# OneWalkman/EDGE-YOLO

Hardware: AMD Instinct MI355X
Metric: images/sec @ 640x640 fp16 (EdgeLine-YOLO detection forward path: backbone + DWT neck + GFLv2 head decode + batched NMS) (higher is better)
Workload: dtype f16; 1 GPU; yolo11n-test.yaml (scale n, nc=80) predict path, 640x640, batch 32/GPU, conf 0.25 iou 0.7 max_det 300, random-init weights, default head biases (DENSE NMS regime: mean detections/img 300); regime=dense, global_batch=32, imgsz=640, nc=80

## Files before the change

edge-yolo_amd/_lib.py:

```python
import ctypes as C
import os

import torch

_HERE = os.path.dirname(os.path.abspath(__file__))
LIB_PATH = os.path.join(_HERE, "csrc", "libedgeyolo_hip.so")

F16, F32 = 0, 1
ACT_NONE, ACT_SILU, ACT_RELU, ACT_SIGMOID = 0, 1, 2, 3
ATTN_AREA_F32, ATTN_AREA_F16, ATTN_AREA_MFMA = 401, 402, 403


class HipLibraryError(RuntimeError):
    pass


class ConvDesc(C.Structure):
    _fields_ = [
        ("dtype", C.c_int32), ("B", C.c_int32), ("H", C.c_int32), ("W", C.c_int32), ("Ho", C.c_int32), ("Wo", C.c_int32),
        ("Cout", C.c_int32), ("k", C.c_int32), ("stride", C.c_int32), ("pad", C.c_int32), ("act", C.c_int32), ("nsrc", C.c_int32),
        ("src", C.c_void_p * 2), ("src_C", C.c_int32 * 2), ("src_cstride", C.c_int32 * 2), ("src_up", C.c_int32 * 2),
        ("w", C.c_void_p), ("bias", C.c_void_p), ("y", C.c_void_p), ("y_cstride", C.c_int32),
        ("res", C.c_void_p), ("res_cstride", C.c_int32), ("out_scale", C.c_float),
        ("addz", C.c_void_p), ("addz_cstride", C.c_int32), ("addz_H", C.c_int32), ("addz_W", C.c_int32), ("ngroup", C.c_int32),
# ... 23 lines not shown
        ("ngroup", C.c_int32), ("src_g", C.c_int64), ("y_g", C.c_int64), ("heads", C.c_int32),
        ("kpad", C.c_int32), ("nt_pack", C.c_int32), ("mt", C.c_int32), ("nti", C.c_int32), ("lds", C.c_int32), ("tile_nti", C.c_int32), ("tile_src_lds", C.c_int32 * 2), ("tile_src_lcs", C.c_int32 * 2), ("tile_y_lds", C.c_int32), ("tile_y_lcs", C.c_int32), ("tile_res_lds", C.c_int32), ("tile_res_lcs", C.c_int32), ("tile_lds_bytes", C.c_int32), ("zsy", C.c_float), ("zsx", C.c_float),
    ]


BLK_CONV, BLK_DW, BLK_DWT, BLK_POOL, BLK_LINATTN = range(5)
_vp, _i, _f, _sz = C.c_void_p, C.c_int, C.c_float, C.c_size_t
SIGNATURES = {
    "ey_last_error": (C.c_char_p, []),
    "ey_version": (_i, []),
    "ey_abi_sizeof": (_sz, [_i]),
    "ey_tune_set": (_i, [C.c_char_p, C.c_long]),
    "ey_tune_get": (C.c_long, [C.c_char_p]),
    "ey_conv_packed_bytes": (_sz, [_i, _i, _i, _i]),
    "ey_conv_pack_weight": (_i, [_i, _i, _i, _i, _vp, _vp, _sz]),
    "ey_conv2d": (_i, [C.POINTER(ConvDesc), _vp]),
    "ey_conv_pw_pair": (_i, [C.POINTER(ConvDesc), C.POINTER(ConvDesc), _vp]),
    "ey_conv_variant": (_i, [_i, _i, _i, _i, _i, _i, C.c_long, _i]),
    "ey_conv_last_variant": (_i, []),
    "ey_conv_pack_nt": (_i, [_i]),
    "ey_conv_chain_klen": (_i, [_i]),
    "ey_conv_chain_kperm": (_i, [_i, _vp, _i]),
    "ey_conv_pw_chain": (_i, [_i, _i, _i, _i, _i, _i, _i, _vp, _i, _vp, _vp, _i, _vp, _vp, _i, _vp, _i, _vp]),
    "ey_conv2d_direct": (_i, [C.POINTER(ConvDirectDesc), _vp]),
    "ey_stem_conv": (_i, [_i, _i, _i, _i, _i, _i, _i, _i, _vp, _vp, _vp, _vp, _i, _vp]),
    "ey_dwconv": (_i, [_i, _i, _i, _i, _i, _i, _i, _vp, _i, _vp, _vp, _vp, _i, _vp]),
    "ey_dsconv": (_i, [_i, _i, _i, _i, _i, _i, _i, _i, _vp, _i, _vp, _vp, _i, _vp, _vp, _vp, _i, _vp, _i, _vp]),
    "ey_dsconv_toeplitz_bytes": (_sz, [_i, _i]),
    "ey_dsconv_pack_toeplitz": (_i, [_i, _i, _vp, _vp, _sz]),
    "ey_dsconv_tz": (_i, [_i, _i, _i, _i, _i, _i, _i, _i, _vp, _i, _vp, _vp, _vp, _i, _vp, _vp, _vp, _i, _vp, _i, _vp]),
    "ey_dsconv_last_variant": (_i, []),
    "ey_conv_pw_conv3s2": (_i, [_i, _i, _i, _i, _vp, _i, _i, _vp, _i, _i, _i, _vp, _vp, _i, _i, _vp, _vp, _i, _vp, _i, _vp]),
    "ey_stem_pair": (_i, [_i, _i, _i, _vp, _vp, _vp, _i, _i, _vp, _vp, _i, _vp, _i, _vp]),
    "ey_dsb_pair": (_i, [_i, _i, _i, _i, _i, _i, _i, _i, _vp, _i, _vp, _vp, _vp, _vp, _vp, _vp, _i, _vp, _i, _vp]),
    "ey_dwt_haar": (_i, [_i, _i, _i, _i, _i, _vp, _i, _vp, _i, _vp]),
    "ey_dwt": (_i, [_i, _i, _i, _i, _i, _i, _vp, _vp, _i, _vp, _i, _vp]),
    "ey_wavelet_z": (_i, [_i, _i, _i, _i, _i, _vp, _i, _vp, C.c_long, _vp, _vp, _vp, _i, _vp]),
    "ey_wavelet_z2": (_i, [_i, _i, _i, _i, _i, _i, _vp, _i, _vp, _vp, _i, _vp, C.c_long, _vp, _vp, _vp, _i, _vp]),
    "ey_sppf_pool": (_i, [_i, _i, _i, _i, _i, _vp, _i, _vp, _vp, _vp, _i, _vp]),
    "ey_copy_nhwc": (_i, [_i, _i, _i, _i, _i, _i, _vp, _i, _vp, _i, _vp]),
    "ey_scale_add_channels": (_i, [_i, _i, _i, _i, _i, _vp, _i, _vp, _vp, _i, _vp, _i, _vp]),
    "ey_avgpool2": (_i, [_i, _i, _i, _i, _i, _vp, _i, _vp, _i, _vp]),
    "ey_dwconv_s2": (_i, [_i, _i, _i, _i, _i, _i, _i, _vp, _i, _vp, _vp, _vp, _i, _vp]),
    "ey_hypergraph_workspace_bytes": (_sz, [_i, _i, _i, _i]),
    "ey_hypergraph_conv": (_i, [_i, _i, _i, _i, _i, _i, _i, _vp, _i, _vp, _i, _vp, _vp, _vp, _vp, _vp, _vp, _vp, _vp, _vp, _vp, _sz, _vp]),
    "ey_nchw_to_nhwc": (_i, [_i, _i, _i, _i, _i, _vp, _vp, _i, _vp]),
    "ey_nhwc_to_nchw": (_i, [_i, _i, _i, _i, _i, _vp, _i, _vp, _vp]),
    "ey_letterbox": (_i, [_i, _vp, _i, _i, _i, _vp, _i, _i, _i, _i, _i, _i, _i, _i, _vp]),
    "ey_copy_linear": (_i, [_vp, _vp, _sz, _vp]),
    "ey_letterbox_batch": (_i, [_i, _vp, _i, _i, _i, _i, C.c_long, _vp, _i, _i, _i, _i, _i, _i, _i, _i, _vp]),
    "ey_linear_attention": (_i, [_i, _i, _i, _i, _i, _vp, _i, _vp, _i, _vp]),
    "ey_softmax_attention": (_i, [_i, _i, _i, _i, _i, _i, _f, _vp, _i, _vp, _i, _vp]),
    "ey_attention_last_variant": (_i, []),
    "ey_area_attention": (_i, [_i, _i, _i, _i, _i, _i, _f, _vp, _i, _vp, _i, _vp, _i, _vp, _i, _vp]),
    "ey_head_decode_last_variant": (_i, []),
    "ey_head_decode": (_i, [_i, _i, _i, _i, _i, _f, _vp, _i, _vp, _i, _vp, _vp, _vp, _vp, _i, _vp, _i, _i, _vp]),
    "ey_head_decode_levels": (_i, [_i, _i, _i, _vp, _vp, _vp, _vp, _vp, _vp, _vp, _i, _vp, _vp, _vp, _vp, _i, _vp, _i, _vp, _vp]),
    "ey_head_decode_levels_xyxy": (_i, [_i, _i, _i, _vp, _vp, _vp, _vp, _vp, _vp, _vp, _i, _vp, _vp, _vp, _vp, _i, _vp, _i, _vp, _vp]),
    "ey_e2e_topk_workspace_bytes": (_sz, [_i, _i, _i]),
    "ey_e2e_topk": (_i, [_i, _i, _i, _vp, _i, _vp, _vp, _vp, _sz, _vp]),
    "ey_block_stage_sizeof": (_sz, []),
    "ey_block_program_bytes": (_sz, [_i]),
    "ey_block_compile": (_i, [C.POINTER(BlockStage), _i, _vp, _sz]),
    "ey_block_run": (_i, [_vp, _i, _i, C.POINTER(C.c_void_p), _i, _vp]),
    "ey_block_tileable": (_i, [C.POINTER(BlockStage), _i]),
    "ey_block_run_tiles": (_i, [_vp, _i, _i, _i, _i, _i, C.POINTER(C.c_void_p), _i, _vp]),
# ... 108 lines not shown
```

edge-yolo_amd/csrc/api.cpp:

```cpp
#include <stdarg.h>
#include <stdio.h>
#include <stddef.h>
#include <string.h>
#include "../../include/edgeyolo_hip.h"
#include "tune.h"

static thread_local char g_err[512] = "";

int ey_set_error(int code, const char* fmt, ...) {
  va_list ap;
  va_start(ap, fmt);
  vsnprintf(g_err, sizeof(g_err), fmt, ap);
  va_end(ap);
  return code;
}

extern "C" const char* ey_last_error(void) { return g_err; }
extern "C" int ey_version(void) { return 1; }
extern "C" size_t ey_abi_sizeof(int which) { return which == 0 ? sizeof(ey_conv_desc) : which == 1 ? sizeof(ey_conv_direct_desc) : 0; }

EyTune g_ey_tune;
#define EY_T(f) {#f, offsetof(EyTune, f)}
static const struct { const char* name; size_t off; } k_tunables[] = {
    EY_T(tiles_per_wave), EY_T(mt2_min_m), EY_T(small_m), EY_T(small_wmb), EY_T(halo_min_c), EY_T(ws_lds_kb), EY_T(ws_wg_cu), EY_T(ws_k3_minnt), EY_T(tile_wlds),
    EY_T(tile_s2_minc), EY_T(tile_s2_minm), EY_T(grid_div), EY_T(c3r), EY_T(tile_minwg), EY_T(tile_flat), EY_T(tile_mink), EY_T(pwr_m), EY_T(pwr_frags), EY_T(pw_m),
    EY_T(pw_waves), EY_T(pw_wmb), EY_T(ds_p), EY_T(tz_kmask), EY_T(tz_minpx), EY_T(ds_strip), EY_T(stem_mfma), EY_T(linattn_mfma), EY_T(softattn_mfma), EY_T(areaattn_mfma), EY_T(c3p), EY_T(c3p_min_m), EY_T(c3p_fast), EY_T(c3s), EY_T(c3s_mt4_m), EY_T(c3s_min_work), EY_T(c3s_cfg), EY_T(nms_fast_k), EY_T(nms_mask_wg), EY_T(sppf_min_wg), EY_T(sppf_cv), EY_T(dsb_pair), EY_T(dsb_max_px), EY_T(dsb_rb), EY_T(dsb_fixed), EY_T(dsb_p2), EY_T(stem_pair), EY_T(pw3), EY_T(pw3_min_px), EY_T(pw3_skew), EY_T(pwn), EY_T(pwn_max_m), EY_T(pwn_ntw), EY_T(pwc), EY_T(xcd_map), EY_T(nms_mask_k)};
static long* tunable(const char* name) {
  if (!name) return nullptr;
  for (const auto& t : k_tunables)
    if (!strcmp(t.name, name)) return (long*)((char*)&g_ey_tune + t.off);
  return nullptr;
}
extern "C" int ey_tune_set(const char* name, long value) {
  long* p = tunable(name);
  if (!p) return ey_set_error(EY_EINVAL, "ey_tune_set: unknown tunable '%s'", name ? name : "(null)");
  *p = value;
  return EY_OK;
}
extern "C" long ey_tune_get(const char* name) {
  const long* p = tunable(name);
  return p ? *p : -1;
}
```

edge-yolo_amd/csrc/dsb.hip:

```cpp
#include "common.h"
#include "tune.h"

struct DsbP {
  int B, H, W, act, add;
  const void* x; int xCs; unsigned xBytes;
  const void* wdw1; const void* wpw1; const float* b1;
  const void* wdw2; const void* wpw2; const float* b2;
  void* y; int yCs;
  int RB, Kpad;
};

#define DSB_SLACK 8

template <int K, int KS, int P, bool LAST>
__device__ __forceinline__ void dsb_stage(const DsbP& p, int b, const f16* s_src, int srcW, int src_row0, const f16* s_w, const void* wpw, const float* bias_g,
                                          int row_lo, int row_hi, f16* s_dst, int dstW, int dst_row0, int dst_pad, const f16* s_res, int resW, int res_row0,
                                          int res_pad) {
  constexpr int C = 32 * KS, NT = 2 * KS, CP = C + 8, NX = P + K - 1;
  const int lane = threadIdx.x & 63, r = lane & 15, g = lane >> 4, wave = threadIdx.x >> 6, nwave = blockDim.x >> 6;
  const int ch0 = g * 4 * NT;
  Vec8<f16> af[KS][NT];
  {
    const __amdgpu_buffer_rsrc_t rw = ey_rsrc(wpw, (unsigned)(16 * NT * p.Kpad * (int)sizeof(f16)));
    const unsigned wvoff = (unsigned)((r * p.Kpad + 8 * g) * (int)sizeof(f16));
#pragma unroll
    for (int ks = 0; ks < KS; ++ks)
#pragma unroll
      for (int nt = 0; nt < NT; ++nt) BufLoad8<f16>::load(af[ks][nt], rw, wvoff, (nt * 16 * p.Kpad + ks * 32) * (int)sizeof(f16));
  }
  float bias[4 * NT];
#pragma unroll
  for (int i = 0; i < 4 * NT; ++i) bias[i] = bias_g ? bias_g[ch0 + i] : 0.f;
  const int WS = (p.W + P - 1) / P;
  const int nstrip = (row_hi - row_lo) * WS;
  for (int unit = wave; unit * 16 < nstrip; unit += nwave) {
    const int si = unit * 16 + r;
    const bool sv = si < nstrip;
    const int sic = sv ? si : nstrip - 1;
    const int ry = sic / WS, x0 = (sic - ry * WS) * P, oy = row_lo + ry;
    Vec8<f16> bf[KS][P];
#pragma unroll
    for (int ks = 0; ks < KS; ++ks) {
      const int cb = ks * 32 + 8 * g;
      float acc[P][8];
#pragma unroll
      for (int q = 0; q < P; ++q)
#pragma unroll
        for (int i = 0; i < 8; ++i) acc[q][i] = 0.f;
      const f16* base = s_src + ((oy - K / 2 - src_row0) * srcW + x0) * CP + cb;
#pragma unroll
      for (int ky = 0; ky < K; ++ky) {
        Vec8<f16> xr[NX];
#pragma unroll
        for (int j = 0; j < NX; ++j) xr[j].load(base + (ky * srcW + j) * CP);
#pragma unroll
        for (int kx = 0; kx < K; ++kx) {
          Vec8<f16> w;
          w.load(s_w + (ky * K + kx) * C + cb);
#pragma unroll
          for (int q = 0; q < P; ++q) ey_fma8_mix(xr[q + kx], w, acc[q]);
        }
      }
#pragma unroll
      for (int q = 0; q < P; ++q)
#pragma unroll
        for (int i = 0; i < 8; ++i) bf[ks][q].set(i, acc[q][i]);
    }
#pragma unroll
    for (int q = 0; q < P; ++q) {
      f32x4 pacc[NT];
#pragma unroll
      for (int nt = 0; nt < NT; ++nt) pacc[nt] = (f32x4)0.f;
#pragma unroll
      for (int ks = 0; ks < KS; ++ks)
#pragma unroll
        for (int nt = 0; nt < NT; ++nt) pacc[nt] = __builtin_amdgcn_mfma_f32_16x16x32_f16(af[ks][nt].v, bf[ks][q].v, pacc[nt], 0, 0, 0);
      const int ox = x0 + q;
      if (!sv || ox >= p.W) continue;
      float v[4 * NT];
#pragma unroll
      for (int nt = 0; nt < NT; ++nt)
#pragma unroll
        for (int j = 0; j < 4; ++j) v[4 * nt + j] = pacc[nt][j] + bias[4 * nt + j];
      ey_act_n(v, p.act);
      if constexpr (!LAST) {
        f16* d = s_dst + ((oy - dst_row0) * dstW + ox + dst_pad) * CP + ch0;
#pragma unroll
        for (int h = 0; h < NT / 2; ++h) {
          Vec8<f16> o;
#pragma unroll
          for (int j = 0; j < 8; ++j) o.set(j, v[8 * h + j]);
          o.store(d + 8 * h);
        }
      } else {
        const long m = ((long)b * p.H + oy) * p.W + ox;
        f16* yp = (f16*)p.y + m * p.yCs + ch0;
        const f16* rp = s_res + ((oy - res_row0) * resW + ox + res_pad) * CP + ch0;
#pragma unroll
        for (int h = 0; h < NT / 2; ++h) {
          if (p.add) {
            Vec8<f16> rr;
            rr.load(rp + 8 * h);
#pragma unroll
            for (int j = 0; j < 8; ++j) v[8 * h + j] += rr.get(j);
          }
          Vec8<f16> o;
#pragma unroll
          for (int j = 0; j < 8; ++j) o.set(j, v[8 * h + j]);
          o.store(yp + 8 * h);
        }
      }
    }
  }
}

template <int K1, int K2, int KS, int P1, int P2>
__global__ __launch_bounds__(512) void dsb_pair_kernel(DsbP p) {
  extern __shared__ __attribute__((aligned(16))) char smem[];
  constexpr int C = 32 * KS, CP = C + 8, CV = C / 8, R1 = K1 / 2, R2 = K2 / 2, PPI = 512 / CV;
  const int RI = p.RB + 2 * (R1 + R2), WI = p.W + 2 * R1, RM = p.RB + 2 * R2, WM = p.W + 2 * R2;
  f16* s_in = reinterpret_cast<f16*>(smem);
  f16* s_mid = s_in + (RI * WI + DSB_SLACK) * CP;
  f16* s_w1 = s_mid + (RM * WM + DSB_SLACK) * CP;
  f16* s_w2 = s_w1 + K1 * K1 * C;
  const int tid = threadIdx.x, b = blockIdx.y, y0 = blockIdx.x * p.RB;
  {
    const __amdgpu_buffer_rsrc_t rx = ey_rsrc(p.x, p.xBytes);
    const int cv = tid % CV, NP = RI * WI, iy0 = y0 - R1 - R2;
    constexpr int U = 4;
    int base = tid / CV;
    bool first = true;
    do {
      Vec8<f16> t[U];
#pragma unroll
      for (int j = 0; j < U; ++j) {
        const int px = base + j * PPI, trow = px / WI, u = px - trow * WI, iy = iy0 + trow, ix = u - R1;
        const bool ok = px < NP && iy >= 0 && iy < p.H && ix >= 0 && ix < p.W;
        BufLoad8<f16>::load(t[j], rx, ok ? (unsigned)((((b * p.H + iy) * p.W + ix) * p.xCs + cv * 8) * (int)sizeof(f16)) : EY_OOB);
      }
      if (first) {
        first = false;
        Vec8<f16> z;
        z.zero();
        for (int v = tid; v < (RM * WM + DSB_SLACK) * CP / 8; v += 512) z.store(s_mid + v * 8);
        for (int v = tid; v < K1 * K1 * CV; v += 512) {
          Vec8<f16> w;
          w.load((const f16*)p.wdw1 + v * 8);
          w.store(s_w1 + v * 8);
        }
        for (int v = tid; v < K2 * K2 * CV; v += 512) {
          Vec8<f16> w;
          w.load((const f16*)p.wdw2 + v * 8);
          w.store(s_w2 + v * 8);
        }
      }
#pragma unroll
      for (int j = 0; j < U; ++j) {
        const int px = base + j * PPI;
        if (px < NP) t[j].store(s_in + px * CP + cv * 8);
      }
      base += U * PPI;
    } while (base < NP);
  }
  __syncthreads();
  {
    const int lo = y0 - R2 < 0 ? 0 : y0 - R2, hi = y0 + p.RB + R2 > p.H ? p.H : y0 + p.RB + R2;
    dsb_stage<K1, KS, P1, false>(p, b, s_in, WI, y0 - R1 - R2, s_w1, p.wpw1, p.b1, lo, hi, s_mid, WM, y0 - R2, R2, nullptr, 0, 0, 0);
  }
  __syncthreads();
  {
    const int hi = y0 + p.RB > p.H ? p.H : y0 + p.RB;
    dsb_stage<K2, KS, P2, true>(p, b, s_mid, WM, y0 - R2, s_w2, p.wpw2, p.b2, y0, hi, nullptr, 0, 0, 0, s_in, WI, y0 - R1 - R2, R1);
  }
}

static size_t dsb_lds_bytes(int W, int C, int k1, int k2, int RB) {
  const int CP = C + 8, r1 = k1 / 2, r2 = k2 / 2;
  return ((size_t)((RB + 2 * (r1 + r2)) * (W + 2 * r1) + DSB_SLACK) + (size_t)((RB + 2 * r2) * (W + 2 * r2) + DSB_SLACK)) * CP * 2 + (size_t)(k1 * k1 + k2 * k2) * C * 2;
}

static int dsb_band_rows(int B, int H, int W, int C, int k1, int k2) {
  static int ncu = 0;
  if (!ncu) {
    int dev = 0;
    hipDeviceProp_t prop;
    if (hipGetDevice(&dev) == hipSuccess && hipGetDeviceProperties(&prop, dev) == hipSuccess) ncu = prop.multiProcessorCount;
    if (ncu < 1) ncu = 256;
  }
  long force = tune().dsb_rb;
  if (force > H) force = H;
  if (force > 0) return dsb_lds_bytes(W, C, k1, k2, (int)force) <= 160 * 1024 ? (int)force : 0;
  int best = 0;
  double best_cost = 0;
  for (int rb = 1; rb <= H; ++rb) {
    if (dsb_lds_bytes(W, C, k1, k2, rb) > 160 * 1024) break;
    const long wgs = (long)B * ((H + rb - 1) / rb);
    const double rounds = (double)((wgs + ncu - 1) / ncu);
    const double cost = rounds * ((rb + 2 * (k2 / 2)) * k1 * k1 + rb * k2 * k2 + (double)tune().dsb_fixed);
    if (!best || cost < best_cost) best = rb, best_cost = cost;
  }
  return best;
}

template <int K1, int K2, int KS, int P1, int P2>
static int dsb_launch(DsbP p, int bands, size_t lds, hipStream_t st) {
  static size_t reserved = 0;
  if (lds > 64 * 1024 && lds > reserved) {
    if (hipFuncSetAttribute((const void*)dsb_pair_kernel<K1, K2, KS, P1, P2>, hipFuncAttributeMaxDynamicSharedMemorySize, (int)lds) != hipSuccess)
      return ey_set_error(EY_ELAUNCH, "dsb_pair: cannot reserve %zu B of LDS", lds);
    reserved = lds;
  }
  hipLaunchKernelGGL((dsb_pair_kernel<K1, K2, KS, P1, P2>), dim3((unsigned)bands, (unsigned)p.B), dim3(512), lds, st, p);
  EY_LAUNCH_CHECK("ey_dsb_pair");
  return EY_OK;
}

extern "C" int ey_dsb_pair(int dtype, int B, int H, int W, int C, int k1, int k2, int act, const void* x, int x_cstride, const void* w_dw1_kkc,
                           const void* w_pw1_packed, const float* bias1, const void* w_dw2_kkc, const void* w_pw2_packed, const float* bias2, int add_residual,
                           void* y, int y_cstride, ey_stream_t stream) {
  EY_CHECK(x && y && w_dw1_kkc && w_pw1_packed && w_dw2_kkc && w_pw2_packed, "dsb_pair: null pointer");
  EY_CHECK(B > 0 && H > 0 && W > 0, "dsb_pair: bad extent");
  EY_CHECK(x_cstride >= C && y_cstride >= C, "dsb_pair: cstride");
  const int es = 2;
  const long xbytes = (((long)B * H * W - 1) * x_cstride + C) * es, ybytes = (((long)B * H * W - 1) * y_cstride + C) * es;
  const bool fits = tune().dsb_pair && dtype == EY_F16 && (C == 32 || C == 64) && k1 == 3 && (k2 == 5 || k2 == 7) && B <= 65535 && xbytes < (1L << 31) &&
                    ybytes < (1L << 31) && (x_cstride * es) % 16 == 0 && ey_aligned(x, 16) && (y_cstride * es) % 16 == 0 && ey_aligned(y, 16) &&
                    ey_aligned(w_dw1_kkc, 16) && ey_aligned(w_dw2_kkc, 16) && ey_aligned(w_pw1_packed, 16) && ey_aligned(w_pw2_packed, 16) &&
                    (long)B * H * W <= tune().dsb_max_px;
  if (!fits) return ey_set_error(EY_EUNSUPPORTED, "dsb_pair: shape outside the fused kernel (f16, C 32/64, k 3 -> 5/7, small maps)");
  const int RB = dsb_band_rows(B, H, W, C, k1, k2);
  if (RB < 1) return ey_set_error(EY_EUNSUPPORTED, "dsb_pair: a one-row band of a %d-wide map does not fit LDS", W);
  DsbP p;
  p.B = B; p.H = H; p.W = W; p.act = act; p.add = add_residual;
  p.x = x; p.xCs = x_cstride; p.xBytes = (unsigned)xbytes;
  p.wdw1 = w_dw1_kkc; p.wpw1 = w_pw1_packed; p.b1 = bias1; p.wdw2 = w_dw2_kkc; p.wpw2 = w_pw2_packed; p.b2 = bias2;
  p.y = y; p.yCs = y_cstride;
  p.RB = RB; p.Kpad = ey_conv_kpad(C, es);
  const int bands = (H + RB - 1) / RB;
  const size_t lds = dsb_lds_bytes(W, C, k1, k2, RB);
  hipStream_t st = (hipStream_t)stream;
  int P2 = (int)tune().dsb_p2;
  if (P2 != 1 && P2 != 2 && P2 != 4) P2 = RB * ((W + 1) / 2) < 64 ? 1 : 2;
#define DSB(KV, KSV)                                                          \
  if (k2 == KV && C == 32 * KSV) {                                            \
    if (P2 == 1) return dsb_launch<3, KV, KSV, 2, 1>(p, bands, lds, st);      \
    if (P2 == 4) return dsb_launch<3, KV, KSV, 2, 4>(p, bands, lds, st);      \
    return dsb_launch<3, KV, KSV, 2, 2>(p, bands, lds, st);                   \
  }
  DSB(5, 1) DSB(7, 1) DSB(5, 2) DSB(7, 2)
#undef DSB
  return ey_set_error(EY_EINVAL, "dsb_pair: k2=%d C=%d", k2, C);
}
```

edge-yolo_amd/csrc/tune.h:

```cpp
#pragma once
struct EyTune {
  long tiles_per_wave = 0;
  long mt2_min_m = 300000;
  long small_m = 100000;
  long small_wmb = 48;
  long halo_min_c = 48;
  long ws_lds_kb = 76;
  long ws_wg_cu = 2;
  long ws_k3_minnt = 0;
  long tile_wlds = 1;
  long tile_s2_minc = 64;
  long tile_s2_minm = 40000;
  long grid_div = 1;
  long c3p = 1;
  long c3p_min_m = 40000;
  long c3p_fast = 1;
  long c3s = 1;
  long c3s_mt4_m = 100000;
  long c3s_min_work = 20000;
  long c3s_cfg = 0;
  long c3r = 1;
  long tile_minwg = 400;
  long tile_flat = 1;
  long tile_mink = 0;
  long pwr_m = 110000;
  long pwr_frags = 24;
  long pw_m = 110000;
  long pw_waves = 3072;
  long pw_wmb = 64;
  long xcd_map = 31;
  long pwc = 1;
  long pwn = 1;
  long pwn_max_m = 110000;
  long pwn_ntw = 0;
  long ds_p = 0;
  long tz_kmask = 168;
  long tz_minpx = 100000;
  long ds_strip = 1;
  long dsb_pair = 1;
  long dsb_max_px = 300000;
  long dsb_rb = 0;
  long dsb_p2 = 0;
  long dsb_fixed = 100;
  long stem_pair = 1;
  long pw3 = 1;
  long pw3_skew = 8;
  long pw3_min_px = 100000;
  long stem_mfma = 1;
  long linattn_mfma = 1;
  long softattn_mfma = 1;
  long areaattn_mfma = 1;
  long sppf_min_wg = 128;
  long sppf_cv = 0;
  long nms_mask_wg = 0;
  long nms_mask_k = 1536;
  long nms_fast_k = 2048;
};
extern EyTune g_ey_tune;
static inline const EyTune& tune() { return g_ey_tune; }
```

include/edgeyolo_hip.h:

```cpp
#ifndef EDGEYOLO_HIP_H
#define EDGEYOLO_HIP_H
#include <stddef.h>
#include <stdint.h>

#ifdef __cplusplus
extern "C" {
#endif

typedef void* ey_stream_t;

enum { EY_F16 = 0, EY_F32 = 1 };
enum { EY_ACT_NONE = 0, EY_ACT_SILU = 1, EY_ACT_RELU = 2, EY_ACT_SIGMOID = 3 };
enum { EY_OK = 0, EY_EINVAL = -1, EY_EUNSUPPORTED = -2, EY_ELAUNCH = -3 };

const char* ey_last_error(void);
int ey_version(void);
size_t ey_abi_sizeof(int which);
int ey_tune_set(const char* name, long value);
long ey_tune_get(const char* name);

typedef struct {
  int32_t dtype;
  int32_t B, H, W;
  int32_t Ho, Wo;
// ... 40 lines not shown
  const float* w_oihw; const float* bias;
  void* y; int32_t y_cstride;
} ey_conv_direct_desc;
int ey_conv2d_direct(const ey_conv_direct_desc* d, ey_stream_t stream);

int ey_stem_conv(int x_dtype, int y_dtype, int B, int Cin, int H, int W, int Cout, int act, const void* x_nchw,
                 const float* w_oihw, const float* bias, void* y, int y_cstride, ey_stream_t stream);

int ey_conv_pw_pair(const ey_conv_desc* first, const ey_conv_desc* second, ey_stream_t stream);

int ey_conv_pw_conv3s2(int dtype, int B, int H, int W, const void* src0, int C0, int cstride0, const void* src1, int C1, int cstride1, int Cmid,
                       const void* w1_packed, const float* bias1, int act1, int Cout, const void* w2_packed, const float* bias2, int act2, void* y,
                       int y_cstride, ey_stream_t stream);

int ey_stem_pair(int B, int H, int W, const void* x_nchw, const float* w0_oihw, const float* bias0, int act0, int C1, const void* w1_packed,
                 const float* bias1, int act1, void* y, int y_cstride, ey_stream_t stream);

int ey_dwconv(int dtype, int B, int H, int W, int C, int k, int act, const void* x, int x_cstride, const void* w_kkc,
              const float* bias, void* y, int y_cstride, ey_stream_t stream);

int ey_dsconv(int dtype, int B, int H, int W, int Cin, int Cout, int k, int act, const void* x, int x_cstride,
              const void* w_dw_kkc, const float* dw_bias, int dw_act, const void* w_pw_packed, const float* bias, void* y, int y_cstride, const void* res,
              int res_cstride, ey_stream_t stream);

size_t ey_dsconv_toeplitz_bytes(int C, int k);
int ey_dsconv_pack_toeplitz(int C, int k, const float* w_dw_kkc_host, void* out_host, size_t out_bytes);
int ey_dsconv_tz(int dtype, int B, int H, int W, int Cin, int Cout, int k, int act, const void* x, int x_cstride,
                 const void* w_dw_kkc, const void* w_dw_toeplitz, const float* dw_bias, int dw_act, const void* w_pw_packed, const float* bias,
                 void* y, int y_cstride, const void* res, int res_cstride, ey_stream_t stream);

int ey_dsb_pair(int dtype, int B, int H, int W, int C, int k1, int k2, int act, const void* x, int x_cstride, const void* w_dw1_kkc,
                const void* w_pw1_packed, const float* bias1, const void* w_dw2_kkc, const void* w_pw2_packed, const float* bias2, int add_residual,
                void* y, int y_cstride, ey_stream_t stream);

int ey_dsconv_last_variant(void);

int ey_dwt_haar(int dtype, int B, int H, int W, int C, const void* x, int x_cstride, void* y, int y_cstride,
                ey_stream_t stream);

int ey_dwt(int dtype, int B, int H, int W, int C, int k, const float* taps, const void* x, int x_cstride, void* y, int y_cstride,
           ey_stream_t stream);

int ey_wavelet_z(int dtype, int B, int H, int W, int C, const void* x, int x_cstride, const void* w_sub_packed, long w_set_stride, const float* b_sub,
                 const void* w_z_packed, void* z, int z_cstride, ey_stream_t stream);
int ey_wavelet_z2(int dtype, int B, int H, int W, int C, int k, const float* taps, int use_ds, const void* w_dw_kkc, const void* x, int x_cstride,
                  const void* w_sub_packed, long w_set_stride, const float* b_sub, const void* w_z_packed, void* z, int z_cstride, ey_stream_t stream);

int ey_sppf_pool(int dtype, int B, int H, int W, int C, const void* x, int x_cstride, void* y1, void* y2, void* y3,
                 int y_cstride, ey_stream_t stream);

int ey_scale_add_channels(int dtype, int B, int H, int W, int C, const void* x, int x_cstride, const float* gamma, const void* t, int t_cstride,
                          void* y, int y_cstride, ey_stream_t stream);

int ey_avgpool2(int dtype, int B, int H, int W, int C, const void* x, int x_cstride, void* y, int y_cstride, ey_stream_t stream);

int ey_dwconv_s2(int dtype, int B, int H, int W, int C, int k, int act, const void* x, int x_cstride, const void* w_kkc, const float* bias,
                 void* y, int y_cstride, ey_stream_t stream);

size_t ey_hypergraph_workspace_bytes(int B, int N, int D, int E);
int ey_hypergraph_conv(int dtype, int B, int N, int D, int E, int heads, int context, const void* x, int x_cstride, void* y, int y_cstride,
                       const float* proto_base, const float* ctx_wT, const float* ctx_b, const float* pre_w, const float* pre_b,
                       const float* edge_wT, const float* edge_b, const void* node_w, const float* node_b, void* workspace,
                       size_t workspace_bytes, ey_stream_t stream);

int ey_copy_nhwc(int dtype, int B, int H, int W, int C, int up, const void* src, int src_cstride, void* dst,
                 int dst_cstride, ey_stream_t stream);
// ... 97 lines not shown
```

Baseline: 28110 images/s.

## Add column-tiled walking-window DSB kernel with ring-buffered LDS and cost planner

Result: no change. 27990 images/s (-0.4%).

```diff
diff --git a/edge-yolo_amd/_lib.py b/edge-yolo_amd/_lib.py
--- a/edge-yolo_amd/_lib.py
+++ b/edge-yolo_amd/_lib.py
@@ -79,6 +79,7 @@
     "ey_dsconv_last_variant": (_i, []),
     "ey_conv_pw_conv3s2": (_i, [_i, _i, _i, _i, _vp, _i, _i, _vp, _i, _i, _i, _vp, _vp, _i, _i, _vp, _vp, _i, _vp, _i, _vp]),
     "ey_stem_pair": (_i, [_i, _i, _i, _vp, _vp, _vp, _i, _i, _vp, _vp, _i, _vp, _i, _vp]),
+    "ey_dsb_pair_plan": (_i, [_i, _i, _i, _i, _i, _vp]),
     "ey_dsb_pair": (_i, [_i, _i, _i, _i, _i, _i, _i, _i, _vp, _i, _vp, _vp, _vp, _vp, _vp, _vp, _i, _vp, _i, _vp]),
     "ey_dwt_haar": (_i, [_i, _i, _i, _i, _i, _vp, _i, _vp, _i, _vp]),
     "ey_dwt": (_i, [_i, _i, _i, _i, _i, _i, _vp, _vp, _i, _vp, _i, _vp]),
diff --git a/edge-yolo_amd/csrc/api.cpp b/edge-yolo_amd/csrc/api.cpp
--- a/edge-yolo_amd/csrc/api.cpp
+++ b/edge-yolo_amd/csrc/api.cpp
@@ -24,7 +24,7 @@
 static const struct { const char* name; size_t off; } k_tunables[] = {
     EY_T(tiles_per_wave), EY_T(mt2_min_m), EY_T(small_m), EY_T(small_wmb), EY_T(halo_min_c), EY_T(ws_lds_kb), EY_T(ws_wg_cu), EY_T(ws_k3_minnt), EY_T(tile_wlds),
     EY_T(tile_s2_minc), EY_T(tile_s2_minm), EY_T(grid_div), EY_T(c3r), EY_T(tile_minwg), EY_T(tile_flat), EY_T(tile_mink), EY_T(pwr_m), EY_T(pwr_frags), EY_T(pw_m),
-    EY_T(pw_waves), EY_T(pw_wmb), EY_T(ds_p), EY_T(tz_kmask), EY_T(tz_minpx), EY_T(ds_strip), EY_T(stem_mfma), EY_T(linattn_mfma), EY_T(softattn_mfma), EY_T(areaattn_mfma), EY_T(c3p), EY_T(c3p_min_m), EY_T(c3p_fast), EY_T(c3s), EY_T(c3s_mt4_m), EY_T(c3s_min_work), EY_T(c3s_cfg), EY_T(nms_fast_k), EY_T(nms_mask_wg), EY_T(sppf_min_wg), EY_T(sppf_cv), EY_T(dsb_pair), EY_T(dsb_max_px), EY_T(dsb_rb), EY_T(dsb_fixed), EY_T(dsb_p2), EY_T(stem_pair), EY_T(pw3), EY_T(pw3_min_px), EY_T(pw3_skew), EY_T(pwn), EY_T(pwn_max_m), EY_T(pwn_ntw), EY_T(pwc), EY_T(xcd_map), EY_T(nms_mask_k)};
+    EY_T(pw_waves), EY_T(pw_wmb), EY_T(ds_p), EY_T(tz_kmask), EY_T(tz_minpx), EY_T(ds_strip), EY_T(stem_mfma), EY_T(linattn_mfma), EY_T(softattn_mfma), EY_T(areaattn_mfma), EY_T(c3p), EY_T(c3p_min_m), EY_T(c3p_fast), EY_T(c3s), EY_T(c3s_mt4_m), EY_T(c3s_min_work), EY_T(c3s_cfg), EY_T(nms_fast_k), EY_T(nms_mask_wg), EY_T(sppf_min_wg), EY_T(sppf_cv), EY_T(dsb_pair), EY_T(dsb_max_px), EY_T(dsb_rb), EY_T(dsb_fixed), EY_T(dsb_form), EY_T(dsb_tw), EY_T(dsb_sr), EY_T(dsb_thr), EY_T(dsb_p2), EY_T(stem_pair), EY_T(pw3), EY_T(pw3_min_px), EY_T(pw3_skew), EY_T(pwn), EY_T(pwn_max_m), EY_T(pwn_ntw), EY_T(pwc), EY_T(xcd_map), EY_T(nms_mask_k)};
 static long* tunable(const char* name) {
   if (!name) return nullptr;
   for (const auto& t : k_tunables)
diff --git a/edge-yolo_amd/csrc/dsb.hip b/edge-yolo_amd/csrc/dsb.hip
--- a/edge-yolo_amd/csrc/dsb.hip
+++ b/edge-yolo_amd/csrc/dsb.hip
@@ -1,5 +1,6 @@
 #include "common.h"
 #include "tune.h"
+#include <string.h>
 
 struct DsbP {
   int B, H, W, act, add;
@@ -8,36 +9,50 @@
   const void* wdw2; const void* wpw2; const float* b2;
   void* y; int yCs;
   int RB, Kpad;
+  int TW, SR;
 };
 
 #define DSB_SLACK 8
 
-template <int K, int KS, int P, bool LAST>
-__device__ __forceinline__ void dsb_stage(const DsbP& p, int b, const f16* s_src, int srcW, int src_row0, const f16* s_w, const void* wpw, const float* bias_g,
-                                          int row_lo, int row_hi, f16* s_dst, int dstW, int dst_row0, int dst_pad, const f16* s_res, int resW, int res_row0,
-                                          int res_pad) {
+struct DsbTile {
+  f16* s;
+  int W, row0, col0, rows;
+};
+
+template <int KS>
+struct DsbW {
+  Vec8<f16> af[KS][2 * KS];
+  float bias[8 * KS];
+  __device__ __forceinline__ void load(const DsbP& p, const void* wpw, const float* bias_g) {
+    constexpr int NT = 2 * KS;
+    const int lane = threadIdx.x & 63, r = lane & 15, g = lane >> 4;
+    const __amdgpu_buffer_rsrc_t rw = ey_rsrc(wpw, (unsigned)(16 * NT * p.Kpad * (int)sizeof(f16)));
+    const unsigned wvoff = (unsigned)((r * p.Kpad + 8 * g) * (int)sizeof(f16));
+#pragma unroll
+    for (int ks = 0; ks < KS; ++ks)
+#pragma unroll
+      for (int nt = 0; nt < NT; ++nt) BufLoad8<f16>::load(af[ks][nt], rw, wvoff, (nt * 16 * p.Kpad + ks * 32) * (int)sizeof(f16));
+#pragma unroll
+    for (int i = 0; i < 4 * NT; ++i) bias[i] = bias_g ? bias_g[g * 4 * NT + i] : 0.f;
+  }
+};
+
+template <int K, int KS, int P, bool LAST, bool RING>
+__device__ __forceinline__ void dsb_stage(const DsbP& p, int b, const DsbTile src, const f16* s_w, const DsbW<KS>& pw, int row_lo, int row_hi, int col_lo,
+                                          int col_hi, const DsbTile dst, const DsbTile res) {
   constexpr int C = 32 * KS, NT = 2 * KS, CP = C + 8, NX = P + K - 1;
   const int lane = threadIdx.x & 63, r = lane & 15, g = lane >> 4, wave = threadIdx.x >> 6, nwave = blockDim.x >> 6;
   const int ch0 = g * 4 * NT;
-  Vec8<f16> af[KS][NT];
-  {
-    const __amdgpu_buffer_rsrc_t rw = ey_rsrc(wpw, (unsigned)(16 * NT * p.Kpad * (int)sizeof(f16)));
-    const unsigned wvoff = (unsigned)((r * p.Kpad + 8 * g) * (int)sizeof(f16));
-#pragma unroll
-    for (int ks = 0; ks < KS; ++ks)
-#pragma unroll
-      for (int nt = 0; nt < NT; ++nt) BufLoad8<f16>::load(af[ks][nt], rw, wvoff, (nt * 16 * p.Kpad + ks * 32) * (int)sizeof(f16));
-  }
-  float bias[4 * NT];
-#pragma unroll
-  for (int i = 0; i < 4 * NT; ++i) bias[i] = bias_g ? bias_g[ch0 + i] : 0.f;
-  const int WS = (p.W + P - 1) / P;
+  const int srcW = src.W;
+  const int WS = (col_hi - col_lo + P - 1) / P;
   const int nstrip = (row_hi - row_lo) * WS;
   for (int unit = wave; unit * 16 < nstrip; unit += nwave) {
     const int si = unit * 16 + r;
     const bool sv = si < nstrip;
     const int sic = sv ? si : nstrip - 1;
-    const int ry = sic / WS, x0 = (sic - ry * WS) * P, oy = row_lo + ry;
+    const int ry = sic / WS, x0 = col_lo + (sic - ry * WS) * P, oy = row_lo + ry;
+    int srow = oy - K / 2 - src.row0;
+    if constexpr (RING) srow %= src.rows;
     Vec8<f16> bf[KS][P];
 #pragma unroll
     for (int ks = 0; ks < KS; ++ks) {
@@ -47,12 +62,17 @@
       for (int q = 0; q < P; ++q)
 #pragma unroll
         for (int i = 0; i < 8; ++i) acc[q][i] = 0.f;
-      const f16* base = s_src + ((oy - K / 2 - src_row0) * srcW + x0) * CP + cb;
+      const f16* base = src.s + ((RING ? 0 : srow * srcW) + x0 - K / 2 - src.col0) * CP + cb;
 #pragma unroll
       for (int ky = 0; ky < K; ++ky) {
         Vec8<f16> xr[NX];
-#pragma unroll
-        for (int j = 0; j < NX; ++j) xr[j].load(base + (ky * srcW + j) * CP);
+        int trow = ky;
+        if constexpr (RING) {
+          trow = srow + ky;
+          if (trow >= src.rows) trow -= src.rows;
+        }
+#pragma unroll
+        for (int j = 0; j < NX; ++j) xr[j].load(base + (trow * srcW + j) * CP);
 #pragma unroll
         for (int kx = 0; kx < K; ++kx) {
           Vec8<f16> w;
@@ -74,17 +94,19 @@
 #pragma unroll
       for (int ks = 0; ks < KS; ++ks)
 #pragma unroll
-        for (int nt = 0; nt < NT; ++nt) pacc[nt] = __builtin_amdgcn_mfma_f32_16x16x32_f16(af[ks][nt].v, bf[ks][q].v, pacc[nt], 0, 0, 0);
+        for (int nt = 0; nt < NT; ++nt) pacc[nt] = __builtin_amdgcn_mfma_f32_16x16x32_f16(pw.af[ks][nt].v, bf[ks][q].v, pacc[nt], 0, 0, 0);
       const int ox = x0 + q;
-      if (!sv || ox >= p.W) continue;
+      if (!sv || ox >= col_hi) continue;
       float v[4 * NT];
 #pragma unroll
       for (int nt = 0; nt < NT; ++nt)
 #pragma unroll
-        for (int j = 0; j < 4; ++j) v[4 * nt + j] = pacc[nt][j] + bias[4 * nt + j];
+        for (int j = 0; j < 4; ++j) v[4 * nt + j] = pacc[nt][j] + pw.bias[4 * nt + j];
       ey_act_n(v, p.act);
       if constexpr (!LAST) {
-        f16* d = s_dst + ((oy - dst_row0) * dstW + ox + dst_pad) * CP + ch0;
+        int drow = oy - dst.row0;
+        if constexpr (RING) drow %= dst.rows;
+        f16* d = dst.s + (drow * dst.W + ox - dst.col0) * CP + ch0;
 #pragma unroll
         for (int h = 0; h < NT / 2; ++h) {
           Vec8<f16> o;
@@ -95,7 +117,9 @@
       } else {
         const long m = ((long)b * p.H + oy) * p.W + ox;
         f16* yp = (f16*)p.y + m * p.yCs + ch0;
-        const f16* rp = s_res + ((oy - res_row0) * resW + ox + res_pad) * CP + ch0;
+        int rrow = oy - res.row0;
+        if constexpr (RING) rrow %= res.rows;
+        const f16* rp = res.s + (rrow * res.W + ox - res.col0) * CP + ch0;
 #pragma unroll
         for (int h = 0; h < NT / 2; ++h) {
           if (p.add) {
@@ -124,6 +148,7 @@
   f16* s_w1 = s_mid + (RM * WM + DSB_SLACK) * CP;
   f16* s_w2 = s_w1 + K1 * K1 * C;
   const int tid = threadIdx.x, b = blockIdx.y, y0 = blockIdx.x * p.RB;
+  const DsbTile t_in = {s_in, WI, y0 - R1 - R2, -R1, RI}, t_mid = {s_mid, WM, y0 - R2, -R2, RM};
   {
     const __amdgpu_buffer_rsrc_t rx = ey_rsrc(p.x, p.xBytes);
     const int cv = tid % CV, NP = RI * WI, iy0 = y0 - R1 - R2;
@@ -165,12 +190,132 @@
   __syncthreads();
   {
     const int lo = y0 - R2 < 0 ? 0 : y0 - R2, hi = y0 + p.RB + R2 > p.H ? p.H : y0 + p.RB + R2;
-    dsb_stage<K1, KS, P1, false>(p, b, s_in, WI, y0 - R1 - R2, s_w1, p.wpw1, p.b1, lo, hi, s_mid, WM, y0 - R2, R2, nullptr, 0, 0, 0);
+    DsbW<KS> pw;
+    pw.load(p, p.wpw1, p.b1);
+    dsb_stage<K1, KS, P1, false, false>(p, b, t_in, s_w1, pw, lo, hi, 0, p.W, t_mid, t_mid);
   }
   __syncthreads();
   {
     const int hi = y0 + p.RB > p.H ? p.H : y0 + p.RB;
-    dsb_stage<K2, KS, P2, true>(p, b, s_mid, WM, y0 - R2, s_w2, p.wpw2, p.b2, y0, hi, nullptr, 0, 0, 0, s_in, WI, y0 - R1 - R2, R1);
+    DsbW<KS> pw;
+    pw.load(p, p.wpw2, p.b2);
+    dsb_stage<K2, KS, P2, true, false>(p, b, t_mid, s_w2, pw, y0, hi, 0, p.W, t_mid, t_in);
+  }
+}
+
+#define DSB_WALK_PF 4
+template <int K1, int K2, int KS, int P1, int P2>
+__global__ __launch_bounds__(512) void dsb_walk_kernel(DsbP p) {
+  extern __shared__ __attribute__((aligned(16))) char smem[];
+  constexpr int C = 32 * KS, CP = C + 8, CV = C / 8, R1 = K1 / 2, R2 = K2 / 2, RH = R1 + R2;
+  const int RS = p.RB, RI = RS + 2 * RH, WI = p.TW + 2 * RH, RM = RS + 2 * R2, WM = p.TW + 2 * R2;
+  f16* s_in = reinterpret_cast<f16*>(smem);
+  f16* s_mid = s_in + (RI * WI + DSB_SLACK) * CP;
+  f16* s_w1 = s_mid + (RM * WM + DSB_SLACK) * CP;
+  f16* s_w2 = s_w1 + K1 * K1 * C;
+  const int tid = threadIdx.x, nthr = blockDim.x, PPI = nthr / CV, cv = tid % CV;
+  const int nsx = (p.W + p.TW - 1) / p.TW, nsy = (p.H + p.SR - 1) / p.SR;
+  const int wi = (int)ey_xcd_block(blockIdx.x, gridDim.x);
+  const int b = wi / (nsx * nsy), ws = wi - b * (nsx * nsy), sy = ws / nsx;
+  const int x0 = (ws - sy * nsx) * p.TW, y0 = sy * p.SR;
+  const int x1 = x0 + p.TW > p.W ? p.W : x0 + p.TW, y1 = y0 + p.SR > p.H ? p.H : y0 + p.SR;
+  const DsbTile t_in = {s_in, WI, y0 - RH, x0 - RH, RI}, t_mid = {s_mid, WM, y0 - R2, x0 - R2, RM};
+  const __amdgpu_buffer_rsrc_t rx = ey_rsrc(p.x, p.xBytes);
+  auto src_off = [&](int px, int np, int row0, int& lds) -> unsigned {
+    const int trow = px / WI, u = px - trow * WI, iy = row0 + trow, ix = x0 - RH + u;
+    lds = (((iy - t_in.row0) % RI) * WI + u) * CP + cv * 8;
+    const bool ok = px < np && iy >= 0 && iy < p.H && ix >= 0 && ix < p.W;
+    return ok ? (unsigned)((((b * p.H + iy) * p.W + ix) * p.xCs + cv * 8) * (int)sizeof(f16)) : EY_OOB;
+  };
+  {
+    const int NP = RI * WI;
+    constexpr int U = 4;
+    int base = tid / CV;
+    bool first = true;
+    do {
+      Vec8<f16> t[U];
+      int lds[U];
+#pragma unroll
+      for (int j = 0; j < U; ++j) BufLoad8<f16>::load(t[j], rx, src_off(base + j * PPI, NP, t_in.row0, lds[j]));
+      if (first) {
+        first = false;
+        Vec8<f16> z;
+        z.zero();
+        for (int v = tid; v < (RM * WM + DSB_SLACK) * CP / 8; v += nthr) z.store(s_mid + v * 8);
+        for (int v = tid; v < K1 * K1 * CV; v += nthr) {
+          Vec8<f16> w;
+          w.load((const f16*)p.wdw1 + v * 8);
+          w.store(s_w1 + v * 8);
+        }
+        for (int v = tid; v < K2 * K2 * CV; v += nthr) {
+          Vec8<f16> w;
+          w.load((const f16*)p.wdw2 + v * 8);
+          w.store(s_w2 + v * 8);
+        }
+      }
+#pragma unroll
+      for (int j = 0; j < U; ++j)
+        if (base + j * PPI < NP) t[j].store(s_in + lds[j]);
+      base += U * PPI;
+    } while (base < NP);
+  }
+  constexpr bool HOIST = KS == 1;
+  DsbW<KS> pw1, pw2;
+  if constexpr (HOIST) {
+    pw1.load(p, p.wpw1, p.b1);
+    pw2.load(p, p.wpw2, p.b2);
+  }
+  const int c_lo = x0 - R2 < 0 ? 0 : x0 - R2, c_hi = x1 + R2 > p.W ? p.W : x1 + R2;
+  const int m_end = y1 + R2 > p.H ? p.H : y1 + R2;
+  __syncthreads();
+  {
+    if constexpr (!HOIST) pw1.load(p, p.wpw1, p.b1);
+    const int lo = y0 - R2 < 0 ? 0 : y0 - R2, hi = y0 + R2 > m_end ? m_end : y0 + R2;
+    dsb_stage<K1, KS, P1, false, true>(p, b, t_in, s_w1, pw1, lo, hi, c_lo, c_hi, t_mid, t_mid);
+  }
+  const int nstep = (y1 - y0 + RS - 1) / RS, NPS = RS * WI;
+  for (int s = 0; s < nstep; ++s) {
+    const int y = y0 + s * RS, nrow0 = y + RS + RH;
+    const bool more = s + 1 < nstep;
+    Vec8<f16> t[DSB_WALK_PF];
+    int lds[DSB_WALK_PF];
+    if (more) {
+#pragma unroll
+      for (int j = 0; j < DSB_WALK_PF; ++j) BufLoad8<f16>::load(t[j], rx, src_off(tid / CV + j * PPI, NPS, nrow0, lds[j]));
+    }
+    {
+      const int lo = y + R2, top = y + RS + R2, hi = top > m_end ? m_end : top;
+      if (top > p.H) {
+        Vec8<f16> z;
+        z.zero();
+        const int zlo = lo > p.H ? lo : p.H, rowv = WM * CP / 8;
+        for (int v = tid; v < (top - zlo) * rowv; v += nthr) {
+          const int zr = v / rowv;
+          z.store(s_mid + ((zlo + zr - t_mid.row0) % RM) * WM * CP + (v - zr * rowv) * 8);
+        }
+      }
+      if constexpr (!HOIST) pw1.load(p, p.wpw1, p.b1);
+      dsb_stage<K1, KS, P1, false, true>(p, b, t_in, s_w1, pw1, lo, hi, c_lo, c_hi, t_mid, t_mid);
+    }
+    __syncthreads();
+    {
+      if constexpr (!HOIST) pw2.load(p, p.wpw2, p.b2);
+      const int hi = y + RS > y1 ? y1 : y + RS;
+      dsb_stage<K2, KS, P2, true, true>(p, b, t_mid, s_w2, pw2, y, hi, x0, x1, t_mid, t_in);
+    }
+    if (more) {
+      if (RS > RH) __syncthreads();
+#pragma unroll
+      for (int j = 0; j < DSB_WALK_PF; ++j)
+        if (tid / CV + j * PPI < NPS) t[j].store(s_in + lds[j]);
+      for (int px = tid / CV + DSB_WALK_PF * PPI; px < NPS; px += PPI) {
+        Vec8<f16> v;
+        int l;
+        BufLoad8<f16>::load(v, rx, src_off(px, NPS, nrow0, l));
+        v.store(s_in + l);
+      }
+    }
+    __syncthreads();
   }
 }
 
@@ -178,39 +323,142 @@
   const int CP = C + 8, r1 = k1 / 2, r2 = k2 / 2;
   return ((size_t)((RB + 2 * (r1 + r2)) * (W + 2 * r1) + DSB_SLACK) + (size_t)((RB + 2 * r2) * (W + 2 * r2) + DSB_SLACK)) * CP * 2 + (size_t)(k1 * k1 + k2 * k2) * C * 2;
 }
-
-static int dsb_band_rows(int B, int H, int W, int C, int k1, int k2) {
-  static int ncu = 0;
-  if (!ncu) {
-    int dev = 0;
-    hipDeviceProp_t prop;
-    if (hipGetDevice(&dev) == hipSuccess && hipGetDeviceProperties(&prop, dev) == hipSuccess) ncu = prop.multiProcessorCount;
-    if (ncu < 1) ncu = 256;
-  }
+static size_t dsb_walk_lds_bytes(int TW, int C, int k1, int k2, int RS) {
+  const int CP = C + 8, rh = k1 / 2 + k2 / 2, r2 = k2 / 2;
+  return ((size_t)((RS + 2 * rh) * (TW + 2 * rh) + DSB_SLACK) + (size_t)((RS + 2 * r2) * (TW + 2 * r2) + DSB_SLACK)) * CP * 2 + (size_t)(k1 * k1 + k2 * k2) * C * 2;
+}
+#define DSB_LDS_MAX (160 * 1024)
+
+static int dsb_ncu() {
+  static int ncu[64];
+  int dev = 0;
+  if (hipGetDevice(&dev) != hipSuccess || dev < 0 || dev >= 64) return 256;
+  if (!ncu[dev]) {
+    int n = 0;
+    if (hipDeviceGetAttribute(&n, hipDeviceAttributeMultiprocessorCount, dev) != hipSuccess || n < 1) n = 256;
+    ncu[dev] = n;
+  }
+  return ncu[dev];
+}
+
+#define DSB_C_PX 0.9
+#define DSB_C_TAP 0.055
+#define DSB_C_STEP 350.0
+#define DSB_C_WG 2500.0
+struct DsbPlan {
+  int form, TW, SR, RS, threads;
+  size_t lds;
+  double cost;
+};
+static double dsb_cost(int B, int H, int W, int C, int k1, int k2, int form, int TW, int SR, int RS, size_t lds, int threads, int ncu) {
+  const int rh = k1 / 2 + k2 / 2, r2 = k2 / 2;
+  const int nseg = (H + SR - 1) / SR, nstrip = (W + TW - 1) / TW, steps = (SR + RS - 1) / RS;
+  const double in_cols = form ? TW + 2 * rh : W, mid_cols = form ? TW + 2 * r2 : W;
+  const double in_px = (double)(SR + 2 * rh) * in_cols, mid_px = (double)(SR + 2 * r2) * mid_cols, out_px = (double)SR * TW;
+  const double wg = (DSB_C_PX * in_px + DSB_C_TAP * (mid_px * k1 * k1 + out_px * k2 * k2)) * (C / 32.0) + DSB_C_STEP * steps + DSB_C_WG;
+  const long wgs = (long)B * nseg * nstrip, slots = (long)ncu * (2 * lds <= DSB_LDS_MAX && threads <= 256 ? 2 : 1);
+  return (double)((wgs + slots - 1) / slots) * wg;
+}
+static int dsb_walk_threads(int TW, int RS, int k2, size_t lds) {
+  long thr = tune().dsb_thr;
+  if (thr == 256 || thr == 512) return (int)thr;
+  return 2 * lds > DSB_LDS_MAX && RS * ((TW + 2 * (k2 / 2) + 1) / 2) > 64 ? 512 : 256;
+}
+static bool dsb_plan_band(int B, int H, int W, int C, int k1, int k2, int ncu, DsbPlan& best) {
   long force = tune().dsb_rb;
   if (force > H) force = H;
-  if (force > 0) return dsb_lds_bytes(W, C, k1, k2, (int)force) <= 160 * 1024 ? (int)force : 0;
-  int best = 0;
-  double best_cost = 0;
+  best.form = -1;
   for (int rb = 1; rb <= H; ++rb) {
-    if (dsb_lds_bytes(W, C, k1, k2, rb) > 160 * 1024) break;
+    const size_t lds = dsb_lds_bytes(W, C, k1, k2, rb);
+    if (lds > DSB_LDS_MAX || (force > 0 && rb > force)) break;
     const long wgs = (long)B * ((H + rb - 1) / rb);
     const double rounds = (double)((wgs + ncu - 1) / ncu);
     const double cost = rounds * ((rb + 2 * (k2 / 2)) * k1 * k1 + rb * k2 * k2 + (double)tune().dsb_fixed);
-    if (!best || cost < best_cost) best = rb, best_cost = cost;
-  }
-  return best;
-}
-
-template <int K1, int K2, int KS, int P1, int P2>
-static int dsb_launch(DsbP p, int bands, size_t lds, hipStream_t st) {
-  static size_t reserved = 0;
-  if (lds > 64 * 1024 && lds > reserved) {
-    if (hipFuncSetAttribute((const void*)dsb_pair_kernel<K1, K2, KS, P1, P2>, hipFuncAttributeMaxDynamicSharedMemorySize, (int)lds) != hipSuccess)
-      return ey_set_error(EY_ELAUNCH, "dsb_pair: cannot reserve %zu B of LDS", lds);
-    reserved = lds;
-  }
-  hipLaunchKernelGGL((dsb_pair_kernel<K1, K2, KS, P1, P2>), dim3((unsigned)bands, (unsigned)p.B), dim3(512), lds, st, p);
+    if (best.form < 0 || force > 0 || cost < best.cost) best = {0, W, rb, rb, 512, lds, cost};
+  }
+  return best.form == 0;
+}
+static bool dsb_plan_walk(int B, int H, int W, int C, int k1, int k2, int ncu, DsbPlan& best) {
+  long ftw = tune().dsb_tw, fsr = tune().dsb_sr, frs = tune().dsb_rb;
+  if (ftw > W) ftw = W;
+  if (fsr > H) fsr = H;
+  best.form = -1;
+  for (int nx = 1; nx <= W; ++nx) {
+    int TW = (W + nx - 1) / nx;
+    if (ftw > 0) TW = (int)ftw;
+    else if (nx > 1 && TW < 16) break;
+    if (dsb_walk_lds_bytes(TW, C, k1, k2, 1) > DSB_LDS_MAX) {
+      if (ftw > 0) {
+        while (TW > 1 && dsb_walk_lds_bytes(TW, C, k1, k2, 1) > DSB_LDS_MAX) --TW;
+      } else continue;
+    }
+    for (int ny = 1, last = 0; ny <= H; ++ny) {
+      int SR = (H + ny - 1) / ny;
+      if (fsr > 0) SR = (int)fsr;
+      if (SR == last) continue;
+      last = SR;
+      for (int RS = (frs > 0 ? (int)(frs > SR ? SR : frs) : (SR < 8 ? SR : 8)); RS >= 1; --RS) {
+        const size_t lds = dsb_walk_lds_bytes(TW, C, k1, k2, RS);
+        if (lds > DSB_LDS_MAX) continue;
+        const int thr = dsb_walk_threads(TW, RS, k2, lds);
+        const DsbPlan c = {1, TW, SR, RS, thr, lds, dsb_cost(B, H, W, C, k1, k2, 1, TW, SR, RS, lds, thr, ncu)};
+        if (best.form < 0 || c.cost < best.cost) best = c;
+        if (frs > 0) break;
+      }
+      if (fsr > 0) break;
+    }
+    if (ftw > 0) break;
+  }
+  return best.form == 1;
+}
+
+static bool dsb_walk_adopted(int B, int H, int W, int C, int k2, int ncu, DsbPlan& plan) {
+  if (!(C == 32 && k2 == 7 && H == 80 && W == 80 && ((long)B * 8) % ncu == 0)) return false;
+  const int TW = 80, SR = 10, RS = 4;
+  plan = {1, TW, SR, RS, 512, dsb_walk_lds_bytes(TW, C, 3, k2, RS), 0.};
+  return true;
+}
+static bool dsb_plan(int B, int H, int W, int C, int k1, int k2, DsbPlan& plan) {
+  const int ncu = dsb_ncu();
+  const long form = tune().dsb_form;
+  struct Memo { long key[10]; DsbPlan plan; };
+  static thread_local Memo memo[16];
+  static thread_local int next = 0;
+  const long key[10] = {B, H, W, C, k2, form, tune().dsb_tw, tune().dsb_sr, tune().dsb_rb, tune().dsb_thr * 1024 + ncu};
+  for (const Memo& m : memo)
+    if (m.key[0] && !memcmp(m.key, key, sizeof(key))) {
+      plan = m.plan;
+      return true;
+    }
+  DsbPlan band, walk;
+  const bool has_band = form != 1 && dsb_plan_band(B, H, W, C, k1, k2, ncu, band);
+  const bool has_walk = form != 0 && dsb_plan_walk(B, H, W, C, k1, k2, ncu, walk);
+  if (form == 2 && !has_band) return false;
+  if (form == 2) {
+    if (!(tune().dsb_rb == 0 && tune().dsb_tw == 0 && tune().dsb_sr == 0 && tune().dsb_thr == 0 && dsb_walk_adopted(B, H, W, C, k2, ncu, plan))) plan = band;
+  } else if (has_band && has_walk) plan = walk.cost < band.cost ? walk : band;
+  else if (has_band) plan = band;
+  else if (has_walk) plan = walk;
+  else return false;
+  Memo& m = memo[next++ & 15];
+  memcpy(m.key, key, sizeof(key));
+  m.plan = plan;
+  return true;
+}
+
+extern "C" int ey_dsb_pair_plan(int B, int H, int W, int C, int k2, int* out6) {
+  EY_CHECK(out6 && B > 0 && H > 0 && W > 0 && (C == 32 || C == 64) && (k2 == 5 || k2 == 7), "dsb_pair_plan: bad argument");
+  DsbPlan plan;
+  if (!dsb_plan(B, H, W, C, 3, k2, plan)) return ey_set_error(EY_EUNSUPPORTED, "dsb_pair_plan: nothing fits LDS");
+  out6[0] = plan.form; out6[1] = plan.TW; out6[2] = plan.SR; out6[3] = plan.RS; out6[4] = plan.threads; out6[5] = (int)plan.lds;
+  return EY_OK;
+}
+
+template <auto Kernel>
+static int dsb_launch(DsbP p, dim3 grid, int threads, size_t lds, hipStream_t st) {
+  if (lds > 64 * 1024 && hipFuncSetAttribute((const void*)Kernel, hipFuncAttributeMaxDynamicSharedMemorySize, (int)lds) != hipSuccess)
+    return ey_set_error(EY_ELAUNCH, "dsb_pair: cannot reserve %zu B of LDS", lds);
+  hipLaunchKernelGGL(Kernel, grid, dim3((unsigned)threads), lds, st, p);
   EY_LAUNCH_CHECK("ey_dsb_pair");
   return EY_OK;
 }
@@ -228,26 +476,46 @@
                     ey_aligned(w_dw1_kkc, 16) && ey_aligned(w_dw2_kkc, 16) && ey_aligned(w_pw1_packed, 16) && ey_aligned(w_pw2_packed, 16) &&
                     (long)B * H * W <= tune().dsb_max_px;
   if (!fits) return ey_set_error(EY_EUNSUPPORTED, "dsb_pair: shape outside the fused kernel (f16, C 32/64, k 3 -> 5/7, small maps)");
-  const int RB = dsb_band_rows(B, H, W, C, k1, k2);
-  if (RB < 1) return ey_set_error(EY_EUNSUPPORTED, "dsb_pair: a one-row band of a %d-wide map does not fit LDS", W);
+  {
+    const uintptr_t xa = (uintptr_t)x, ya = (uintptr_t)y;
+    if (xa < ya + (uintptr_t)ybytes && ya < xa + (uintptr_t)xbytes) {
+      const long cs = x_cstride, d = (((long)(ya / es) - (long)(xa / es)) % cs + cs) % cs;
+      if (x_cstride != y_cstride || d < C || cs - d < C) return ey_set_error(EY_EUNSUPPORTED, "dsb_pair: y overlaps x (only disjoint channel windows of one buffer may)");
+    }
+  }
+  DsbPlan plan;
+  if (!dsb_plan(B, H, W, C, k1, k2, plan)) return ey_set_error(EY_EUNSUPPORTED, "dsb_pair: not even a one-row tile of a %d-wide map fits LDS", W);
   DsbP p;
   p.B = B; p.H = H; p.W = W; p.act = act; p.add = add_residual;
   p.x = x; p.xCs = x_cstride; p.xBytes = (unsigned)xbytes;
   p.wdw1 = w_dw1_kkc; p.wpw1 = w_pw1_packed; p.b1 = bias1; p.wdw2 = w_dw2_kkc; p.wpw2 = w_pw2_packed; p.b2 = bias2;
   p.y = y; p.yCs = y_cstride;
-  p.RB = RB; p.Kpad = ey_conv_kpad(C, es);
-  const int bands = (H + RB - 1) / RB;
-  const size_t lds = dsb_lds_bytes(W, C, k1, k2, RB);
+  p.RB = plan.RS; p.TW = plan.TW; p.SR = plan.SR; p.Kpad = ey_conv_kpad(C, es);
   hipStream_t st = (hipStream_t)stream;
   int P2 = (int)tune().dsb_p2;
-  if (P2 != 1 && P2 != 2 && P2 != 4) P2 = RB * ((W + 1) / 2) < 64 ? 1 : 2;
-#define DSB(KV, KSV)                                                          \
-  if (k2 == KV && C == 32 * KSV) {                                            \
-    if (P2 == 1) return dsb_launch<3, KV, KSV, 2, 1>(p, bands, lds, st);      \
-    if (P2 == 4) return dsb_launch<3, KV, KSV, 2, 4>(p, bands, lds, st);      \
-    return dsb_launch<3, KV, KSV, 2, 2>(p, bands, lds, st);                   \
-  }
-  DSB(5, 1) DSB(7, 1) DSB(5, 2) DSB(7, 2)
+  if (P2 != 1 && P2 != 2 && P2 != 4) P2 = plan.RS * ((plan.TW + 1) / 2) < 64 ? 1 : 2;
+  if (plan.form == 1) {
+    const long wgs = (long)B * ((H + plan.SR - 1) / plan.SR) * ((W + plan.TW - 1) / plan.TW);
+    if (wgs >= (1L << 31)) return ey_set_error(EY_EUNSUPPORTED, "dsb_pair: too many tiles");
+    const dim3 grid((unsigned)wgs);
+#define DSB(KV, KSV)                                                                                            \
+  if (k2 == KV && C == 32 * KSV) {                                                                              \
+    if (P2 == 1) return dsb_launch<dsb_walk_kernel<3, KV, KSV, 2, 1>>(p, grid, plan.threads, plan.lds, st);     \
+    if (P2 == 4) return dsb_launch<dsb_walk_kernel<3, KV, KSV, 2, 4>>(p, grid, plan.threads, plan.lds, st);     \
+    return dsb_launch<dsb_walk_kernel<3, KV, KSV, 2, 2>>(p, grid, plan.threads, plan.lds, st);                  \
+  }
+    DSB(5, 1) DSB(7, 1) DSB(5, 2) DSB(7, 2)
 #undef DSB
+  } else {
+    const dim3 grid((unsigned)((H + plan.RS - 1) / plan.RS), (unsigned)B);
+#define DSB(KV, KSV)                                                                               \
+  if (k2 == KV && C == 32 * KSV) {                                                                 \
+    if (P2 == 1) return dsb_launch<dsb_pair_kernel<3, KV, KSV, 2, 1>>(p, grid, 512, plan.lds, st); \
+    if (P2 == 4) return dsb_launch<dsb_pair_kernel<3, KV, KSV, 2, 4>>(p, grid, 512, plan.lds, st); \
+    return dsb_launch<dsb_pair_kernel<3, KV, KSV, 2, 2>>(p, grid, 512, plan.lds, st);              \
+  }
+    DSB(5, 1) DSB(7, 1) DSB(5, 2) DSB(7, 2)
+#undef DSB
+  }
   return ey_set_error(EY_EINVAL, "dsb_pair: k2=%d C=%d", k2, C);
 }
diff --git a/edge-yolo_amd/csrc/tune.h b/edge-yolo_amd/csrc/tune.h
--- a/edge-yolo_amd/csrc/tune.h
+++ b/edge-yolo_amd/csrc/tune.h
@@ -39,7 +39,11 @@
   long ds_strip = 1;
   long dsb_pair = 1;
   long dsb_max_px = 300000;
+  long dsb_form = 2;
   long dsb_rb = 0;
+  long dsb_tw = 0;
+  long dsb_sr = 0;
+  long dsb_thr = 0;
   long dsb_p2 = 0;
   long dsb_fixed = 100;
   long stem_pair = 1;
diff --git a/include/edgeyolo_hip.h b/include/edgeyolo_hip.h
--- a/include/edgeyolo_hip.h
+++ b/include/edgeyolo_hip.h
@@ -96,6 +96,7 @@
 int ey_dsb_pair(int dtype, int B, int H, int W, int C, int k1, int k2, int act, const void* x, int x_cstride, const void* w_dw1_kkc,
                 const void* w_pw1_packed, const float* bias1, const void* w_dw2_kkc, const void* w_pw2_packed, const float* bias2, int add_residual,
                 void* y, int y_cstride, ey_stream_t stream);
+int ey_dsb_pair_plan(int B, int H, int W, int C, int k2, int* out6);
 
 int ey_dsconv_last_variant(void);
 
```
